# naver/deep-image-retrieval

Hardware: AMD Instinct MI355X
Metric: images/sec descriptor extraction (resnet101-GeM, 1024x1024) (higher is better)
Workload: dtype fp16p

## Files before the change

deep-image-retrieval_amd/csrc/conv_c3c1.hip:

```cpp
#include "dir_common.h"
#include "conv_device.h"
#include "conv_igemm.h"

namespace dir {

template <class DT, int P, bool DS, int P2, bool WP3 = false, bool WP1 = false>
__global__ void __launch_bounds__(512) conv_c3c1_kernel(const ConvArgs a) {
    static_assert(P == 64 || P == 128, "planes");
    static_assert(P2 == P || (P == 64 && P2 == 128), "conv1' width");
    static_assert(!DS || (P == 64 && P2 == 64), "the downsample form is layer1's: 64 + 64 input channels");
    static_assert((!WP3 && !WP1) || P == 64, "paired weights: layer1's seams");
    constexpr int KW = P + (DS ? 64 : 0);
    constexpr int KA = KW + (DS && WP3 ? 64 : 0);
    constexpr int C4 = 4 * P;
    constexpr int BM = 64, NT = 512;
    constexpr int CW = C4 / 8;
    constexpr int TA = CW / 32;
    constexpr int KSA = KA / 16;
    constexpr int KSW = KW / 16;
    constexpr int XBUF = BM * KA * 2;
    constexpr int NX = XBUF / 16 / NT;
    constexpr int EROW = 32 * 4 + 16;
    constexpr int EPI_OFF = 2 * XBUF;
    constexpr int OUT_OFF = EPI_OFF + 8 * 32 * EROW;
    constexpr int OUTB = BM * C4 * 2;
    constexpr int BIAS_OFF = OUT_OFF + OUTB;
    constexpr int KSB = (C4 / 2) / 16;
    typedef typename DT::frag_t frag_t;
    static_assert(NX >= 1 && XBUF % (16 * NT) == 0, "tile split");

    extern __shared__ __attribute__((aligned(16))) char smem[];

    const int tid = threadIdx.x;
    const int lane = tid & 63;
    const int wave = __builtin_amdgcn_readfirstlane(tid >> 6);
    const int lrow = lane & 31, lhi = lane >> 5;

    const __amdgpu_buffer_rsrc_t rsrc_x = buffer_rsrc(a.x, a.x_bytes);
    const __amdgpu_buffer_rsrc_t rsrc_x2 =
        buffer_rsrc(DS ? a.x2 : a.x, DS ? (uint32_t)((size_t)a.M * 128) : a.x_bytes);
    const __amdgpu_buffer_rsrc_t rsrc_x2l =
        buffer_rsrc(DS && WP3 ? a.x2_lo : a.x, DS && WP3 ? (uint32_t)((size_t)a.M * 128) : a.x_bytes);
    const uint32_t y_bytes = (uint32_t)((size_t)a.M * C4 * 2);
    const uint32_t y2_bytes = (uint32_t)((size_t)a.M * P2 * 2);
    const __amdgpu_buffer_rsrc_t rsrc_r = buffer_rsrc(a.res, y_bytes);
    const __amdgpu_buffer_rsrc_t rsrc_y = buffer_rsrc(a.y, y_bytes);
    const __amdgpu_buffer_rsrc_t rsrc_y2 = buffer_rsrc(a.y2, y2_bytes);

    const int mt = (a.M + BM - 1) / BM;
    const int per = gridDim.x;
    int tile = blockIdx.x;
    if (tile >= mt) return;
    Ovf<DT> ovf;
    const int n_wave = wave * CW;

    frag_t w3[TA][KSW], w3l[WP3 ? TA : 1][WP3 ? KSW : 1];
#pragma unroll
    for (int i = 0; i < TA; ++i)
#pragma unroll
        for (int ks = 0; ks < KSW; ++ks) {
            w3[i][ks] = *(const DIR_GLOBAL frag_t*)(a.w + (size_t)(n_wave + i * 32 + lrow) * KW + ks * 16 + 8 * lhi);
            if (WP3)
                w3l[i][ks] = *(const DIR_GLOBAL frag_t*)(a.w_lo + (size_t)(n_wave + i * 32 + lrow) * KW + ks * 16 + 8 * lhi);
        }
    constexpr bool WIDE = P2 == 128;
    const int nt = WIDE ? (wave & 3) : (wave & 1);
    const int kh = wave >> 2;
    const int jb = WIDE ? 0 : ((wave >> 1) & 1);
    frag_t w1[KSB], w1l[WP1 ? KSB : 1];
#pragma unroll
    for (int ks = 0; ks < KSB; ++ks) {
        w1[ks] = *(const DIR_GLOBAL frag_t*)(a.w2 + (size_t)(nt * 32 + lrow) * C4 + kh * (C4 / 2) + ks * 16 + 8 * lhi);
        if (WP1)
            w1l[ks] = *(const DIR_GLOBAL frag_t*)(a.w2_lo + (size_t)(nt * 32 + lrow) * C4 + kh * (C4 / 2) + ks * 16 + 8 * lhi);
    }
#pragma unroll
    for (int i = 0; i < TA; ++i)
#pragma unroll
        for (int ks = 0; ks < KSW; ++ks) {
// ... 7 lines not shown
    }

    const int spix = (tid >> 3) & 63, sslot = tid & 7;
    const int sdst = spix * 128 + ((sslot ^ ((spix >> 1) & 7)) << 4);
    const int lswz = (lane >> 1) & 7;
    const int lbase = lrow * 128;
    const int ecol = (lane & 3) * 8, erow = lane >> 2;
    float* const sbias3 = (float*)(smem + BIAS_OFF);
    float* const sbias1 = sbias3 + C4;
    for (int i = tid; i < C4; i += NT) sbias3[i] = a.bias[i];
    if (tid < P2) sbias1[tid] = a.bias2[tid];
    char* const ebase = smem + EPI_OFF + wave * (32 * EROW);
    char* const pbase = smem + EPI_OFF + (wave ^ 4) * (32 * EROW);
    char* const otile = smem + OUT_OFF;

    auto load_x = [&](int t, u32x4_t* xr) {
        const int m = t * BM + spix;
        const uint32_t base = m < a.M ? (uint32_t)((m * P + sslot * 8) * 2) : kOOB;
        if (DS) {
            xr[0] = __builtin_amdgcn_raw_buffer_load_b128(rsrc_x, base, 0, 0);
            xr[1] = __builtin_amdgcn_raw_buffer_load_b128(rsrc_x2, base, 0, 0);
            if (WP3) xr[NX - 1] = __builtin_amdgcn_raw_buffer_load_b128(rsrc_x2l, base, 0, 0);
        } else {
#pragma unroll
            for (int i = 0; i < NX; ++i) xr[i] = __builtin_amdgcn_raw_buffer_load_b128(rsrc_x, base, i * 128, 0);
        }
    };
    auto store_x = [&](const u32x4_t* xr, char* buf) {
#pragma unroll
        for (int i = 0; i < NX; ++i) *(u32x4_t*)(buf + i * (BM * 128) + sdst) = xr[i];
    };
    const uint32_t ncol2 = (uint32_t)((n_wave + ecol) * 2);
    auto row_off = [&](int m) { return m < a.M ? (uint32_t)m * (uint32_t)(C4 * 2) + ncol2 : kOOB; };
    auto load_res = [&](int t, int j, u32x4_t* r) {
#pragma unroll
        for (int i = 0; i < TA; ++i)
#pragma unroll
            for (int pass = 0; pass < 2; ++pass)
                r[i * 2 + pass] = __builtin_amdgcn_raw_buffer_load_b128(
                    rsrc_r, row_off(t * BM + j * 32 + pass * 16 + erow), i * 64, 0);
    };

    u32x4_t xr[NX];
    load_x(tile, xr);
    int cur = 0;
    u32x4_t rres0[TA * 2], rres1[TA * 2];
    if (!DS) load_res(tile, 0, rres0);
    store_x(xr, smem);
    __syncthreads();
    for (;;) {
        const bool more = tile + per < mt;
        const int next = more ? tile + per : tile;
        load_x(next, xr);
        const int m0 = tile * BM;
        if (!DS) load_res(tile, 1, rres1);
        const char* xb = smem + cur * XBUF;

#pragma unroll
        for (int j = 0; j < 2; ++j) {
            f32x16_t acc[TA];
#pragma unroll
            for (int i = 0; i < TA; ++i)
#pragma unroll
                for (int e = 0; e < 16; ++e) acc[i][e] = 0.f;
#pragma unroll
            for (int ks = 0; ks < KSA; ++ks) {
                const frag_t xf = *(const frag_t*)(xb + (ks >> 2) * (BM * 128) + j * (32 * 128) + lbase +
                                                   (((2 * (ks & 3) + lhi) ^ lswz) << 4));
                const int kw = ks < KSW ? ks : ks - 4;
#pragma unroll
                for (int i = 0; i < TA; ++i) {
                    acc[i] = DT::mfma32(w3[i][kw], xf, acc[i]);
                    if (WP3 && ks < KSW) acc[i] = DT::mfma32(w3l[i][ks], xf, acc[i]);
                }
                if ((ks & 3) == 3) __builtin_amdgcn_sched_barrier(0);
            }
            if (!DS) {
#pragma unroll
                for (int q = 0; q < TA * 2; ++q) {
                    if (j == 0) {
                        asm volatile("" : "+v"(rres0[q]));
                    } else {
                        asm volatile("" : "+v"(rres1[q]));
                    }
                }
            }
#pragma unroll
            for (int i = 0; i < TA; ++i) {
#pragma unroll
                for (int g = 0; g < 4; ++g) {
                    const f32x4_t v = {acc[i][4 * g + 0], acc[i][4 * g + 1], acc[i][4 * g + 2], acc[i][4 * g + 3]};
                    *(f32x4_t*)(ebase + lrow * EROW + (8 * g + 4 * lhi) * 4) = v;
                }
                wave_lds_sync();
                const float* const bz = sbias3 + n_wave + i * 32 + ecol;
                const f32x4_t b0 = *(const f32x4_t*)bz, b1 = *(const f32x4_t*)(bz + 4);
#pragma unroll
                for (int pass = 0; pass < 2; ++pass) {
                    const int mrow = pass * 16 + erow;
                    const f32x4_t f0 = *(const f32x4_t*)(ebase + mrow * EROW + ecol * 4);
                    const f32x4_t f1 = *(const f32x4_t*)(ebase + mrow * EROW + ecol * 4 + 16);
                    float v[8] = {f0[0] + b0[0], f0[1] + b0[1], f0[2] + b0[2], f0[3] + b0[3],
                                  f1[0] + b1[0], f1[1] + b1[1], f1[2] + b1[2], f1[3] + b1[3]};
                    if (!DS) {
                        const u32x4_t rv = j == 0 ? rres0[i * 2 + pass] : rres1[i * 2 + pass];
                        add_res8<DT>(v, rv);
                    }
                    if (a.relu) relu8(v);
                    u32x4_t ov;
#pragma unroll
                    for (int e = 0; e < 4; ++e) ov[e] = DT::pack(v[2 * e], v[2 * e + 1]);
                    __builtin_amdgcn_raw_buffer_store_b128(ov, rsrc_y, row_off(m0 + j * 32 + mrow), i * 64, 0);
                    ovf.see(ov);
                    const int n = n_wave + i * 32 + ecol, p = j * 32 + mrow;
                    *(u32x4_t*)(otile + (n >> 6) * (BM * 128) + p * 128 + ((((n & 63) >> 3) ^ ((p >> 1) & 7)) << 4)) = ov;
                }
                wave_lds_sync();
            }
            if (!DS && j == 0) load_res(next, 0, rres0);
        }
        __syncthreads();

        {
            constexpr int NJ = WIDE ? 2 : 1;
            f32x16_t acc1[NJ];
#pragma unroll
            for (int jj = 0; jj < NJ; ++jj)
#pragma unroll
                for (int e = 0; e < 16; ++e) acc1[jj][e] = 0.f;
#pragma unroll
            for (int ks = 0; ks < KSB; ++ks) {
                const int kb = kh * (C4 / 128) + (ks >> 2);
#pragma unroll
                for (int jj = 0; jj < NJ; ++jj) {
                    const int j = WIDE ? jj : jb;
                    const frag_t of = *(const frag_t*)(otile + kb * (BM * 128) + j * (32 * 128) + lbase +
                                                       (((2 * (ks & 3) + lhi) ^ lswz) << 4));
                    acc1[jj] = DT::mfma32(w1[ks], of, acc1[jj]);
                    if (WP1) acc1[jj] = DT::mfma32(w1l[ks], of, acc1[jj]);
                }
                if ((ks & 3) == 3) __builtin_amdgcn_sched_barrier(0);
            }
            const int give = WIDE ? (1 - kh) : 0;
            const bool gives = WIDE || kh == 1;
            const bool finishes = WIDE || kh == 0;
// ... 32 lines not shown
                    const int mrow = pass * 16 + erow;
                    const f32x4_t f0 = *(const f32x4_t*)(ebase + mrow * EROW + ecol * 4);
                    const f32x4_t f1 = *(const f32x4_t*)(ebase + mrow * EROW + ecol * 4 + 16);
                    float v[8] = {f0[0] + b0[0], f0[1] + b0[1], f0[2] + b0[2], f0[3] + b0[3],
                                  f1[0] + b1[0], f1[1] + b1[1], f1[2] + b1[2], f1[3] + b1[3]};
                    if (a.relu2) relu8(v);
                    const u32x4_t ov = pack8<DT>(v);
                    const int m = m0 + j * 32 + mrow;
                    const uint32_t off = m < a.M ? (uint32_t)m * (uint32_t)(P2 * 2) + (uint32_t)((nt * 32 + ecol) * 2) : kOOB;
                    __builtin_amdgcn_raw_buffer_store_b128(ov, rsrc_y2, off, 0, 0);
                    ovf.see(ov);
                }
            }
        }
        if (!more) break;
        store_x(xr, smem + (cur ^ 1) * XBUF);
        tile = next;
        cur ^= 1;
        __syncthreads();
    }
    ovf.flush(a.ovf);
}

bool conv_c3c1_admissible(const ConvArgs& a) {
    const bool ds = a.x2 != nullptr;
#ifdef DIR_EXPERIMENTS
    if (a.Cin == 256) return conv_seam3_admissible(a);
#endif
    return a.R == 1 && a.S == 1 && a.stride == 1 && a.pad == 0 && a.H == a.OH && a.W == a.OW &&
           (a.Cin == 64 || a.Cin == 128) && a.Cout == 4 * a.Cin && (ds ? (a.res == nullptr && a.Cin == 64 && a.Cin2 == 64)
                                                                       : a.res != nullptr) &&
           a.w2 != nullptr && a.bias2 != nullptr && a.y2 != nullptr &&
           (a.Cout2 == a.Cin || (!ds && a.Cin == 64 && a.Cout2 == 128)) && (long)a.M * a.Cout < (1L << 30) &&
           ((!a.w_lo && !a.w2_lo && !a.x2_lo) ||
            (a.Cin == 64 && a.w_lo && (a.w2_lo || a.Cout2 == 128) && (ds ? a.x2_lo != nullptr : a.x2_lo == nullptr)));
}

template <class DT, int P, bool DS, int P2 = P, bool WP3 = false, bool WP1 = false>
static hipError_t launch_c3c1(const ConvArgs& a, hipStream_t stream) {
    constexpr int XBUF = 64 * (P + (DS ? 64 : 0) + (DS && WP3 ? 64 : 0)) * 2;
    constexpr int LDS = 2 * XBUF + 8 * 32 * (32 * 4 + 16) + 64 * 4 * P * 2 + (4 * P + P2) * 4;
    static_assert(LDS <= 160 * 1024, "LDS budget");
    auto kern = conv_c3c1_kernel<DT, P, DS, P2, WP3, WP1>;
    static std::atomic<uint64_t> attr_done{0};
    if (hipError_t e = ensure_dynamic_lds((const void*)kern, LDS, attr_done); e != hipSuccess) return e;
    ConvArgs b = a;
    b.x_bytes = (uint32_t)((size_t)a.M * a.Cin * 2);
    const int mt = (a.M + 63) / 64;
    const int ncu = cu_count();
    hipLaunchKernelGGL(kern, dim3(mt < ncu ? mt : ncu), dim3(512), LDS, stream, b);
    return hipGetLastError();
}

hipError_t conv_c3c1_launch(const ConvArgs& a, int dtype, hipStream_t stream) {
#ifdef DIR_EXPERIMENTS
    if (a.Cin == 256) return conv_seam3_launch(a, dtype, stream);
#endif
    if (a.x2 && !env().no_c3c1lc && conv_c3c1ds_lc_admissible(a)) return conv_c3c1ds_lc_launch(a, dtype, stream);
    if (a.w_lo) {
        if (dtype != DIR_FP16) return hipErrorInvalidValue;
        if (a.x2) return a.w2_lo ? launch_c3c1<FP16, 64, true, 64, true, true>(a, stream) : hipErrorInvalidValue;
        if (a.Cout2 == 128)
            return a.w2_lo ? launch_c3c1<FP16, 64, false, 128, true, true>(a, stream)
                           : launch_c3c1<FP16, 64, false, 128, true, false>(a, stream);
        return a.w2_lo ? launch_c3c1<FP16, 64, false, 64, true, true>(a, stream) : hipErrorInvalidValue;
    }
    if (a.x2)
        return dtype == DIR_BF16 ? launch_c3c1<BF16, 64, true>(a, stream) : launch_c3c1<FP16, 64, true>(a, stream);
    if (a.Cin == 128)
        return dtype == DIR_BF16 ? launch_c3c1<BF16, 128, false>(a, stream) : launch_c3c1<FP16, 128, false>(a, stream);
    if (a.Cout2 == 128)
        return dtype == DIR_BF16 ? launch_c3c1<BF16, 64, false, 128>(a, stream) : launch_c3c1<FP16, 64, false, 128>(a, stream);
    return dtype == DIR_BF16 ? launch_c3c1<BF16, 64, false>(a, stream) : launch_c3c1<FP16, 64, false>(a, stream);
}

}
```

deep-image-retrieval_amd/csrc/conv_igemm.h:

```cpp
#pragma once
#include "dir_common.h"

namespace dir {

struct ConvArgs {
    const uint16_t* x;
    const uint16_t* w;
    const float* bias;
    const uint16_t* res;
    uint16_t* y;
    int B, H, W, Cin, OH, OW, Cout;
    int R, S, stride, pad, relu;
    int M;
    int Ktot;
    int T;
    int ksplit;
    float* partial;
    const uint16_t* w2;
    const float* bias2;
    uint16_t* y2;
    int Cout2, relu2;
    const uint16_t* x2;
    int Cin2;
    int H2, W2, stride2;
    uint32_t x2_bytes;
    int* ovf;
    const uint16_t* x_lo;
    const uint16_t* x2_lo;
    const uint16_t* w_lo;
    const uint16_t* w_pw;
    const uint16_t* w_s2;
    const uint16_t* w2_lo;
    const uint16_t* res_lo;
    uint16_t* y_lo;
    int tiles_m, tiles_n;
    uint32_t x_bytes, w_bytes;
    int rev_m;
    int no_xcd_map;
    int flat;
    uint32_t div_ohw_mul, div_ohw_shr;
    uint32_t div_ow_mul, div_ow_shr;
};

inline void fastdiv_init(uint32_t d, uint32_t& mul, uint32_t& shr) {
    if (d <= 1) {
        mul = 0;
        shr = 0;
        return;
    }
    uint32_t l = 0;
    while ((1ull << l) < d) ++l;
    mul = (uint32_t)(((1ull << (31 + l)) + d - 1) / d);
    shr = l - 1;
}
// ... 79 lines not shown
```

deep-image-retrieval_amd/csrc/dir_common.h:

```cpp
#pragma once
#include <hip/hip_runtime.h>
#include <stdint.h>
#include <string.h>
#include <atomic>
#include <string>

#include "../../include/dir_engine.h"

namespace dir {

typedef __attribute__((ext_vector_type(8))) __bf16 bf16x8_t;
typedef __attribute__((ext_vector_type(8))) _Float16 f16x8_t;
typedef __attribute__((ext_vector_type(16))) float f32x16_t;
typedef __attribute__((ext_vector_type(4))) float f32x4_t;
typedef __attribute__((ext_vector_type(4))) uint32_t u32x4_t;
typedef __attribute__((ext_vector_type(2))) uint32_t u32x2_t;
typedef __attribute__((ext_vector_type(2))) float f32x2_t;
typedef __attribute__((ext_vector_type(2))) __bf16 bf16x2_t;
typedef __attribute__((ext_vector_type(2))) _Float16 f16x2_t;

#define DIR_GLOBAL __attribute__((address_space(1)))
#define DIR_LDS __attribute__((address_space(3)))

void set_error(const std::string& msg);
int fail(int code, const std::string& msg);

#define DIR_HIP_CHECK(expr)                                                                \
    do {                                                                                   \
        hipError_t _e = (expr);                                                            \
        if (_e != hipSuccess)                                                              \
            return ::dir::fail(DIR_ERR_HIP, std::string(#expr) + ": " + hipGetErrorString(_e)); \
    } while (0)

struct Env {
    bool c3c1_off = false, c3c1_force = false;
    bool no_ds_seam = false, no_dual = false;
    bool rev_conv1 = false, rev_conv3 = false;
    bool unfused_stem = false, stem_v1 = false;
    bool no_patchlc = false, no_wreg = false, no_patchw = false, no_x3 = false, no_patchs = false;
    bool patchw_pack = false, no_patchw_pack = false;
    bool small_k2 = false;
    bool no_patchs2 = false;
    bool x3_k2048 = false;
    bool lc1x1 = false;
    bool no_c3c1lc = false;
    bool no_smallmap = false;
    bool no_wregd = false;
    bool no_patchw_lc = false;
    bool no_xcdmap = false;
    bool no_pair_patch = false, pair_acts = false;
    int pair_stages = 1;
    bool sim_v1 = false, sim_exact = false;
    bool experiments = false;
    bool no_inplace = false;
    bool no_stem_u8 = false;
    bool stem_pair_old = false;
    bool stem_u8_prep = false;
    bool stem_u8_wg8 = false;
    int stem_u8_seg = 0;
};
const Env& env();
void reload_env();

__host__ __device__ inline uint16_t f32_to_bf16_bits(float f) {
    uint32_t u;
    memcpy(&u, &f, 4);
    if ((u & 0x7fffffffu) > 0x7f800000u) return (uint16_t)((u >> 16) | 0x40);
    u += 0x7fffu + ((u >> 16) & 1u);
    return (uint16_t)(u >> 16);
}
__host__ __device__ inline float bf16_bits_to_f32(uint16_t h) {
    uint32_t u = ((uint32_t)h) << 16;
    float f;
    memcpy(&f, &u, 4);
    return f;
}
__host__ __device__ inline uint16_t f32_to_f16_bits(float f) {
    _Float16 h = (_Float16)f;
    uint16_t b;
    memcpy(&b, &h, 2);
    return b;
}
__host__ __device__ inline float f16_bits_to_f32(uint16_t b) {
    _Float16 h;
    memcpy(&h, &b, 2);
    return (float)h;
}
// ... 122 lines not shown
```

deep-image-retrieval_amd/csrc/engine.h:

```cpp
#pragma once
#include <map>
#include <string>
#include <vector>

#include "conv_f32.h"
#include "conv_igemm.h"
#include "pointwise.h"

namespace dir {

struct HostTensor {
    std::vector<int64_t> shape;
    std::vector<float> data;
};

struct ConvLayer {
    std::string name;
    std::string wkey;
    std::string bnprefix;
    int Cin = 0, Cout = 0, R = 1, S = 1, stride = 1, pad = 0;
    bool relu = false;
    bool stem = false;
    uint16_t* d_w = nullptr;
    float* d_wf = nullptr;
// ... 41 lines not shown
    std::vector<dir::ConvLayer> convs;
    std::vector<dir::BlockDef> blocks;
    int feat_dim = 0;
    int x4_dim = 0;
    int head_dim = 0;
    int x4_block = -1;
    int conv1x5 = -1, conv3c4 = -1;
    float gem_p = 3.f;
    float gem_p4 = 3.f;
    float* d_fc_w = nullptr;
    float* d_fc_b = nullptr;
    int* d_ovf = nullptr;
    uint16_t* d_stem_u8_w = nullptr;
    uint16_t* d_stem_u8_w_lo = nullptr;
    float* d_stem_u8_bias = nullptr;
    float* d_stem_u8_corr = nullptr;
    int fold_stem_u8(dir::ConvLayer& L, const float* w, const float* scale, const float* bias);
    bool profiling = false;
    bool prof_paused = false;
    std::vector<dir::ProfSlot> prof;
    size_t prof_used = 0;
    bool tuning = false;

    int build_graph();
    int finalize(int dtype);
    int plan(int B, int H, int W, dir::Plan* p) const;
    int forward(const void* img, int B, int H, int W, int fmt, float* desc_out, void* feat_out,
                int* fh, int* fw, int* fc, void* ws, size_t ws_bytes, hipStream_t stream);
    int forward_f32(const void* img, int B, int H, int W, int fmt, float* desc_out, void* feat_out, int* fh, int* fw,
                    int* fc, char* base, const dir::Plan& p, hipStream_t stream);
    int run_conv_f32(dir::ConvLayer& L, const float* x, const float* res, float* y, int B, int H, int W, int OH, int OW,
                     hipStream_t stream);
    int run_conv(dir::ConvLayer& L, const uint16_t* x, const uint16_t* res, uint16_t* y, int B,
                 int H, int W, int OH, int OW, hipStream_t stream, bool rev_m = false);
    int run_conv_pair(dir::ConvLayer& L, const uint16_t* x, const uint16_t* x_lo, const uint16_t* res,
                      const uint16_t* res_lo, uint16_t* y, uint16_t* y_lo, int B, int H, int W, int OH, int OW,
                      hipStream_t stream, const uint16_t* x2 = nullptr, const uint16_t* x2_lo = nullptr);
    int forward_pair_head(const void* img, int B, int H, int W, int fmt, char* base, const dir::Plan& p,
                          hipStream_t stream, uint16_t** cur, int* h, int* w, size_t* next_block);
    int forward_pair_stem(const void* img, int B, int H, int W, int fmt, char* base, const dir::Plan& p, hipStream_t stream);
    int run_seam(dir::ConvLayer& c3, dir::ConvLayer& c1, const uint16_t* t2, const uint16_t* res, uint16_t* y,
                 uint16_t* t1, int B, int H, int W, hipStream_t stream, int* used,
                 const uint16_t* block_in = nullptr, const uint16_t* block_in_lo = nullptr);
    int run_conv_dual(dir::ConvLayer& c3, const dir::ConvLayer& ds, const uint16_t* t2, const uint16_t* xin,
                      uint16_t* y, int B, int Hin, int Win, int OH, int OW, hipStream_t stream, int* used, bool dry);
    dir::Env sw;
    float* splitk_scratch = nullptr;
    int prof_begin(const std::string& name, const std::string& kernel, double flops, double bytes,
                   hipStream_t stream);
    int prof_end(hipStream_t stream);
    int overflow(hipStream_t stream, int* overflowed);
    void release();
};
```

deep-image-retrieval_amd/csrc/engine.hip:

```cpp
#include "engine.h"

#include <math.h>
#include <algorithm>

namespace dir {

static thread_local std::string g_err;
void set_error(const std::string& msg) { g_err = msg; }
int fail(int code, const std::string& msg) {
    g_err = msg;
    return code;
}
const char* last_error() { return g_err.c_str(); }


static Env read_env() {
    Env e;
    auto on = [](const char* k) { return getenv(k) != nullptr; };
    const char* mode = getenv("DIRTORCH_AMD_C3C1");
    e.c3c1_off = mode && mode[0] == '0';
    e.c3c1_force = mode && mode[0] == 'f';
    e.no_ds_seam = on("DIRTORCH_AMD_NO_DS_SEAM");
    e.no_dual = on("DIRTORCH_AMD_NO_DUAL");
    e.rev_conv1 = on("DIRTORCH_AMD_REV_CONV1");
    e.rev_conv3 = on("DIRTORCH_AMD_REV_CONV3");
    e.unfused_stem = on("DIRTORCH_AMD_UNFUSED_STEM");
    e.stem_v1 = on("DIRTORCH_AMD_STEM_V1");
    e.no_patchlc = on("DIRTORCH_AMD_NO_PATCHLC");
    e.no_wreg = on("DIRTORCH_AMD_NO_WREG");
    e.no_wregd = on("DIRTORCH_AMD_NO_WREGD");
    e.no_smallmap = on("DIRTORCH_AMD_NO_SMALLMAP");
    e.no_c3c1lc = on("DIRTORCH_AMD_NO_C3C1LC");
    e.lc1x1 = on("DIRTORCH_AMD_LC1X1");
    e.x3_k2048 = on("DIRTORCH_AMD_X3_K2048");
    e.no_patchs2 = on("DIRTORCH_AMD_NO_PATCHS2");
    e.small_k2 = on("DIRTORCH_AMD_SMALL_K2");
    e.patchw_pack = on("DIRTORCH_AMD_PATCHW_PACK");
    e.no_patchw_pack = on("DIRTORCH_AMD_NO_PATCHW_PACK");
    e.no_patchw = on("DIRTORCH_AMD_NO_PATCHW");
    e.no_x3 = on("DIRTORCH_AMD_NO_X3");
    e.no_patchs = on("DIRTORCH_AMD_NO_PATCHS");
    e.no_patchw_lc = on("DIRTORCH_AMD_NO_PATCHW_LC");
    e.no_xcdmap = on("DIRTORCH_AMD_NO_XCDMAP");
    e.no_pair_patch = on("DIRTORCH_AMD_NO_PAIR_PATCH");
    e.pair_acts = on("DIRTORCH_AMD_PAIR_ACTS");
    if (const char* s = getenv("DIRTORCH_AMD_PAIR_STAGES")) e.pair_stages = atoi(s);
    e.sim_v1 = on("DIRTORCH_AMD_SIM_V1");
    e.sim_exact = on("DIRTORCH_AMD_SIM_EXACT");
    e.experiments = on("DIRTORCH_AMD_EXPERIMENTS");
    e.no_inplace = on("DIRTORCH_AMD_NO_INPLACE");
    e.no_stem_u8 = on("DIRTORCH_AMD_NO_STEM_U8");
    e.stem_u8_wg8 = on("DIRTORCH_AMD_STEM_U8_WG8");
    e.stem_u8_prep = on("DIRTORCH_AMD_STEM_U8_PREP");
    e.stem_pair_old = on("DIRTORCH_AMD_STEM_PAIR_OLD");
    if (const char* s = getenv("DIRTORCH_AMD_STEM_U8_SEG")) e.stem_u8_seg = atoi(s);
    return e;
}
static Env g_env[2];
static std::atomic<int> g_env_cur{-1};
static std::atomic_flag g_env_lock = ATOMIC_FLAG_INIT;
static void publish_env() {
    while (g_env_lock.test_and_set(std::memory_order_acquire)) {
    }
    const int cur = g_env_cur.load(std::memory_order_relaxed);
    const int nxt = cur < 0 ? 0 : 1 - cur;
    g_env[nxt] = read_env();
    g_env_cur.store(nxt, std::memory_order_release);
    g_env_lock.clear(std::memory_order_release);
}
const Env& env() {
    int cur = g_env_cur.load(std::memory_order_acquire);
    if (cur < 0) {
        static const bool once = (publish_env(), true);
        (void)once;
        cur = g_env_cur.load(std::memory_order_acquire);
    }
    return g_env[cur];
}
void reload_env() { publish_env(); }

static inline size_t align_up(size_t v, size_t a = 256) { return (v + a - 1) / a * a; }

__global__ void fill_noise_kernel(uint16_t* p, long n, int dtype) {
// ... 404 lines not shown
    }
    p->splitk = take(kSplitKMaxBytes);
    p->pooled = take((size_t)B * head_dim * 4);
    p->fcout = take((size_t)B * std::max(desc.out_dim, head_dim) * 4);
    p->total = off;
    return DIR_OK;
}

int dir_engine::prof_begin(const std::string& name, const std::string& kernel, double flops,
                           double bytes, hipStream_t stream) {
    if (!profiling || prof_paused) return DIR_OK;
    if (prof_used == prof.size()) {
        ProfSlot s;
        DIR_HIP_CHECK(hipEventCreate(&s.start));
        DIR_HIP_CHECK(hipEventCreate(&s.stop));
        prof.push_back(s);
    }
    ProfSlot& s = prof[prof_used];
    s.name = name;
    s.kernel = kernel;
    s.flops = flops;
    s.bytes = bytes;
    DIR_HIP_CHECK(hipEventRecord(s.start, stream));
    return DIR_OK;
}
int dir_engine::prof_end(hipStream_t stream) {
    if (!profiling || prof_paused) return DIR_OK;
    DIR_HIP_CHECK(hipEventRecord(prof[prof_used].stop, stream));
    ++prof_used;
    return DIR_OK;
}

int dir_engine::run_conv(ConvLayer& L, const uint16_t* x, const uint16_t* res, uint16_t* y, int B,
                         int H, int W, int OH, int OW, hipStream_t stream, bool rev_m) {
    if (dtype == DIR_FP16P && L.d_w_lo && !L.stem)
        return run_conv_pair(L, x, nullptr, res, nullptr, y, nullptr, B, H, W, OH, OW, stream);
    ConvArgs a;
    memset(&a, 0, sizeof(a));
    a.rev_m = rev_m ? 1 : 0;
    a.x = x;
    a.w = L.d_w;
    a.w_s2 = L.d_w_s2;
    a.w_pw = env().no_patchw_pack ? nullptr : L.d_w_pw;
    a.bias = L.d_bias;
    a.res = res;
    a.y = y;
    a.B = B;
    a.H = H;
    a.W = W;
    a.OH = OH;
    a.OW = OW;
    a.Cout = L.Cout;
    if (L.stem) {
        a.Cin = 16;
        a.R = a.S = 4;
        a.stride = 1;
        a.pad = 2;
    } else {
        a.Cin = L.Cin;
        a.R = L.R;
        a.S = L.S;
        a.stride = L.stride;
        a.pad = L.pad;
    }
    a.relu = L.relu ? 1 : 0;
    a.ovf = d_ovf;
    a.partial = splitk_scratch;
    a.M = B * OH * OW;
    a.Ktot = a.R * a.S * a.Cin;
    a.T = a.Ktot / 64;
    const double macs = (double)a.M * L.Cout * (double)(L.R * L.S * L.Cin);
    const double bytes = 2.0 * ((double)B * H * W * a.Cin + (double)a.M * L.Cout * (res ? 2 : 1) +
                                (double)L.Cout * a.Ktot);

    int variant = -1;
    auto it = L.tuned.find(a.M);
    if (it != L.tuned.end()) variant = it->second;
    if (tuning && it == L.tuned.end()) {
        hipEvent_t e0, e1;
        DIR_HIP_CHECK(hipEventCreate(&e0));
        DIR_HIP_CHECK(hipEventCreate(&e1));
        float best = 1e30f;
        for (int v = 0; v < conv_variant_count(); ++v) {
            a.ksplit = 0;
            if (!conv_variant_admissible(v, a)) continue;
            a.ksplit = conv_splitk_factor(v, a);
            int rc = conv_launch(a, kdtype(), v, stream);
            if (rc != DIR_OK) return rc;
            float ms = 1e30f;
            for (int round = 0; round < 2; ++round) {
                DIR_HIP_CHECK(hipEventRecord(e0, stream));
                for (int rep = 0; rep < 3; ++rep) {
                    rc = conv_launch(a, kdtype(), v, stream);
                    if (rc != DIR_OK) return rc;
                }
                DIR_HIP_CHECK(hipEventRecord(e1, stream));
                DIR_HIP_CHECK(hipEventSynchronize(e1));
                float t = 0.f;
                DIR_HIP_CHECK(hipEventElapsedTime(&t, e0, e1));
                ms = t < ms ? t : ms;
            }
            if (ms < best) {
                best = ms;
                variant = v;
            }
        }
        (void)hipEventDestroy(e0);
        (void)hipEventDestroy(e1);
        L.tuned[a.M] = variant;
    }
    a.ksplit = 0;
    if (variant >= 0 && !conv_variant_admissible(variant, a)) {
        L.tuned.erase(a.M);
        variant = -1;
    }
    if (variant < 0) variant = conv_pick_variant(a);
    a.ksplit = conv_splitk_factor(variant, a);
    int rc = DIR_OK;
    if (profiling && !prof_paused)
        rc = prof_begin(L.name, std::string("conv_igemm<") + conv_variant(variant).name +
                                    (a.ksplit > 1 ? "/k" + std::to_string(a.ksplit) : "") + ">",
                        2.0 * macs, bytes, stream);
    if (rc != DIR_OK) return rc;
    rc = conv_launch(a, kdtype(), variant, stream);
    if (rc != DIR_OK) return rc;
    return prof_end(stream);
}

int dir_engine::run_conv_pair(ConvLayer& L, const uint16_t* x, const uint16_t* x_lo, const uint16_t* res,
                              const uint16_t* res_lo, uint16_t* y, uint16_t* y_lo, int B, int H, int W, int OH, int OW,
                              hipStream_t stream, const uint16_t* x2, const uint16_t* x2_lo) {
    if (!L.d_w_lo) return fail(DIR_ERR_STATE, "paired conv on a layer without a lo weight plane: " + L.name);
    if (x2 && !L.d_w_ds_lo) return fail(DIR_ERR_STATE, "two-source paired conv without concatenated weights: " + L.name);
    ConvArgs a;
    memset(&a, 0, sizeof(a));
    a.x = x;
    a.x_lo = x_lo;
    a.w = L.d_w;
    a.w_lo = L.d_w_lo;
    a.bias = L.d_bias;
    a.res = res;
    a.res_lo = res_lo;
    a.y = y;
    a.y_lo = y_lo;
    a.B = B;
    a.H = H;
    a.W = W;
// ... 114 lines not shown
        if (desc.bottleneck) {
            rc = run_conv_pair(convs[bd.conv1], x, x_lo, nullptr, nullptr, t1, t1_lo, B, h, w, h, w, stream);
            if (rc != DIR_OK) return rc;
            rc = run_conv_pair(convs[bd.conv2], t1, t1_lo, nullptr, nullptr, t2, t2_lo, B, h, w, oh, ow, stream);
            if (rc != DIR_OK) return rc;
            if (fuse_ds)
                rc = run_conv_pair(convs[bd.conv3], t2, t2_lo, nullptr, nullptr, pp[nxt], nullptr, B, oh, ow, oh, ow, stream,
                                   x, x_lo);
            else
                rc = run_conv_pair(convs[bd.conv3], t2, t2_lo, resid, resid_lo, pp[nxt], nullptr, B, oh, ow, oh, ow, stream);
            if (rc != DIR_OK) return rc;
        } else {
            rc = run_conv_pair(convs[bd.conv1], x, x_lo, nullptr, nullptr, t1, t1_lo, B, h, w, oh, ow, stream);
            if (rc != DIR_OK) return rc;
            rc = run_conv_pair(convs[bd.conv2], t1, t1_lo, resid, resid_lo, pp[nxt], nullptr, B, oh, ow, oh, ow, stream);
            if (rc != DIR_OK) return rc;
        }
        cur = nxt;
        h = oh;
        w = ow;
    }
    *cur_out = pp[cur];
    *h_out = h;
    *w_out = w;
    *next_block = nb;
    return DIR_OK;
}

static constexpr long kSeamMinTiles = 2048;
static constexpr long kSeam3MinTiles = 768;

int dir_engine::run_seam(ConvLayer& c3, ConvLayer& c1, const uint16_t* t2, const uint16_t* res, uint16_t* y,
                         uint16_t* t1, int B, int H, int W, hipStream_t stream, int* used,
                         const uint16_t* block_in, const uint16_t* block_in_lo) {
    *used = 0;
    if (sw.c3c1_off) return DIR_OK;
    ConvArgs a;
    memset(&a, 0, sizeof(a));
    a.x = t2;
    a.w = c3.d_w;
    a.w_lo = c3.d_w_lo;
    a.w2_lo = c1.d_w_lo;
    a.bias = c3.d_bias;
    a.res = res;
    if (block_in) {
        if (!c3.d_w_ds || c3.Cin != 64) return DIR_OK;
        a.w = c3.d_w_ds;
        a.w_lo = c3.d_w_ds_lo;
        a.bias = c3.d_bias_ds;
        a.res = nullptr;
        a.x2 = block_in;
        a.x2_lo = block_in_lo;
        a.Cin2 = 64;
        if ((c3.d_w_lo != nullptr) != (a.w_lo != nullptr)) return DIR_OK;
    }
    a.y = y;
    a.B = B;
    a.H = a.OH = H;
    a.W = a.OW = W;
    a.Cin = c3.Cin;
    a.Cout = c3.Cout;
    a.R = c3.R;
    a.S = c3.S;
    a.stride = c3.stride;
    a.pad = c3.pad;
    a.relu = c3.relu ? 1 : 0;
    a.M = B * H * W;
    a.Ktot = a.Cin;
    a.w2 = c1.d_w;
    a.bias2 = c1.d_bias;
    a.y2 = t1;
    a.Cout2 = c1.Cout;
    a.relu2 = c1.relu ? 1 : 0;
    a.ovf = d_ovf;
    if (c1.R != 1 || c1.S != 1 || c1.stride != 1 || c1.pad != 0 || c1.Cin != c3.Cout || !conv_c3c1_admissible(a))
        return DIR_OK;
    if (!sw.c3c1_force && (a.M + 63) / 64 < (a.Cin == 256 ? kSeam3MinTiles : kSeamMinTiles)) return DIR_OK;
    if (a.Cin == 256 && !sw.experiments) return DIR_OK;
    const double macs = (double)a.M * ((double)c3.Cout * (c3.Cin + a.Cin2) + (double)c1.Cout * c1.Cin);
    const double bytes = 2.0 * ((double)a.M * (c3.Cin + a.Cin2 * (block_in_lo ? 2 : 1) + (block_in ? 1.0 : 2.0) * c3.Cout + c1.Cout) +
                                (double)c3.Cout * (c3.Cin + a.Cin2) * (a.w_lo ? 2 : 1) + (double)c1.Cout * c1.Cin * (a.w2_lo ? 2 : 1));
    int rc = DIR_OK;
    if (profiling && !prof_paused)
        rc = prof_begin(c3.name.substr(0, c3.name.rfind('.')) + (block_in ? ".ds+c3c1" : ".c3c1"),
                        (c3.Cin == 256 ? "conv_seam3<" : "conv_c3c1<") + std::to_string(c3.Cin) + (block_in ? ",ds" : "") +
                            (a.w_lo ? ",wp>" : ">"),
                        2.0 * macs, bytes, stream);
    if (rc != DIR_OK) return rc;
    hipError_t e = conv_c3c1_launch(a, kdtype(), stream);
    if (e != hipSuccess) return fail(DIR_ERR_HIP, std::string("conv_c3c1 launch: ") + hipGetErrorString(e));
    *used = 1;
    return prof_end(stream);
}

int dir_engine::run_conv_dual(ConvLayer& c3, const ConvLayer& ds, const uint16_t* t2, const uint16_t* xin,
                              uint16_t* y, int B, int Hin, int Win, int OH, int OW, hipStream_t stream, int* used,
                              bool dry) {
    *used = 0;
    if (!c3.d_w_ds || sw.no_dual || c3.d_w_lo) return DIR_OK;
    ConvArgs a;
    memset(&a, 0, sizeof(a));
    a.x = t2;
    a.w = c3.d_w_ds;
    a.bias = c3.d_bias_ds;
    a.y = y;
    a.B = B;
    a.H = a.OH = OH;
    a.W = a.OW = OW;
    a.Cin = c3.Cin;
    a.Cout = c3.Cout;
    a.R = a.S = 1;
    a.stride = 1;
    a.relu = c3.relu ? 1 : 0;
    a.ovf = d_ovf;
    a.M = B * OH * OW;
    a.x2 = xin;
    a.Cin2 = ds.Cin;
    a.H2 = Hin;
    a.W2 = Win;
    a.stride2 = ds.stride;
    a.Ktot = a.Cin + a.Cin2;
    a.T = a.Ktot / 64;
    const int variant = conv_pick_dual_variant(a);
    if (variant < 0) return DIR_OK;
    *used = 1;
    if (dry) return DIR_OK;
    const double macs = (double)a.M * c3.Cout * (double)a.Ktot;
    const double bytes = 2.0 * ((double)a.M * (c3.Cin + ds.Cin + c3.Cout) + (double)c3.Cout * a.Ktot);
    int rc = DIR_OK;
    if (profiling && !prof_paused)
        rc = prof_begin(c3.name.substr(0, c3.name.rfind('.')) + ".ds+conv3",
                        std::string("conv_igemm<") + conv_variant(variant).name + "/dual>", 2.0 * macs, bytes, stream);
    if (rc != DIR_OK) return rc;
    rc = conv_launch(a, kdtype(), variant, stream);
    if (rc != DIR_OK) return rc;
    return prof_end(stream);
}

int dir_engine::forward(const void* img, int B, int H, int W, int fmt, float* desc_out,
                        void* feat_out, int* fh, int* fw, int* fc, void* ws, size_t ws_bytes,
                        hipStream_t stream) {
    if (!finalized) return fail(DIR_ERR_STATE, "forward before finalize");
    int cur_dev = -1;
    DIR_HIP_CHECK(hipGetDevice(&cur_dev));
    if (cur_dev != device)
        return fail(DIR_ERR_STATE, "forward: the current HIP device (" + std::to_string(cur_dev) +
                                       ") is not the engine's device (" + std::to_string(device) + ")");
    Plan p;
    int rc = plan(B, H, W, &p);
    if (rc != DIR_OK) return rc;
    if (!ws || ws_bytes < p.total)
        return fail(DIR_ERR_WORKSPACE, "workspace too small: need " + std::to_string(p.total) +
                                           " bytes, got " + std::to_string(ws_bytes));
// ... 35 lines not shown
        } else {
            const long n = (long)B * p.H2 * p.W2 * 16;
            hipLaunchKernelGGL(fill_noise_kernel, dim3((unsigned)((n + 255) / 256)), dim3(256), 0, stream,
                               s2d, n, kd);
            DIR_HIP_CHECK(hipGetLastError());
        }
        if (sw.unfused_stem) {
            rc = run_conv(convs[0], s2d, nullptr, stem, B, p.H2, p.W2, p.OH1, p.OW1, stream);
            if (rc != DIR_OK) return rc;
            rc = prof_begin("maxpool", "maxpool_3x3s2", 0,
                            2.0 * ((double)B * p.OH1 * p.OW1 * 64 + (double)B * p.PH * p.PW * 64), stream);
            if (rc != DIR_OK) return rc;
            rc = maxpool_3x3s2(stem, cur, B, p.OH1, p.OW1, 64, kd, stream);
            if (rc != DIR_OK) return rc;
            if ((rc = prof_end(stream)) != DIR_OK) return rc;
        } else {
            rc = prof_begin("conv1+maxpool", "stem_pool", 2.0 * B * p.OH1 * p.OW1 * 64.0 * 147.0,
                            2.0 * ((double)B * p.H2 * p.W2 * 16 + (double)B * p.PH * p.PW * 64 + 64 * 256),
                            stream);
            if (rc != DIR_OK) return rc;
            rc = stem_pool_launch(s2d, convs[0].d_w, convs[0].d_bias, cur, B, p.H2, p.W2, p.OH1, p.OW1,
                                  kd, stream, d_ovf);
            if (rc != DIR_OK) return rc;
            if ((rc = prof_end(stream)) != DIR_OK) return rc;
        }
        h = p.PH;
        w = p.PW;
    }

    uint16_t* const pp[2] = {(uint16_t*)(base + p.bufA), (uint16_t*)(base + p.bufB)};
    uint16_t* x4 = nullptr;
    int h4 = 0, w4 = 0;
    bool t1_ready = false;
    for (size_t bi = first_block; bi < blocks.size(); ++bi) {
        BlockDef& bd = blocks[bi];
        const int oh = conv_out(h, 3, bd.stride, 1), ow = conv_out(w, 3, bd.stride, 1);
        const bool keep = (int)bi == x4_block;
        nxt = keep ? (uint16_t*)(base + p.x4) : (cur == pp[0] ? pp[1] : pp[0]);
        if (!sw.no_inplace && desc.bottleneck && bd.down < 0 && !keep && !tuning && convs[bd.conv3].Cin >= 256) nxt = cur;
        const uint16_t* resid = cur;
        const bool seam_next = desc.bottleneck && bi + 1 < blocks.size() && !tuning;
        bool ds_in_seam = false;
        if (bd.down >= 0 && seam_next && convs[bd.conv3].d_w_ds && convs[bd.conv3].Cin == 64 &&
            convs[bd.down].Cin == 64 && convs[bd.down].stride == 1 && convs[blocks[bi + 1].conv1].Cout == 64 &&
            convs[blocks[bi + 1].conv1].Cin == convs[bd.conv3].Cout) {
            ds_in_seam = !sw.c3c1_off && !sw.no_ds_seam && (sw.c3c1_force || ((long)B * oh * ow + 63) / 64 >= kSeamMinTiles) &&
                         (long)B * oh * ow * convs[bd.conv3].Cout < (1L << 30);
        }
        int ds_dual = 0;
        if (bd.down >= 0 && !ds_in_seam && desc.bottleneck && !tuning && !cur_lo) {
            rc = run_conv_dual(convs[bd.conv3], convs[bd.down], t2, cur, nxt, B, h, w, oh, ow, stream, &ds_dual, true);
            if (rc != DIR_OK) return rc;
        }
        if (bd.down >= 0 && !ds_in_seam && !ds_dual) {
            rc = cur_lo ? run_conv_pair(convs[bd.down], cur, cur_lo, nullptr, nullptr, ds, nullptr, B, h, w, oh, ow, stream)
                        : run_conv(convs[bd.down], cur, nullptr, ds, B, h, w, oh, ow, stream);
            if (rc != DIR_OK) return rc;
            resid = ds;
        }
        if (desc.bottleneck) {
            if (!t1_ready) {
                rc = cur_lo ? run_conv_pair(convs[bd.conv1], cur, cur_lo, nullptr, nullptr, t1, nullptr, B, h, w, h, w, stream)
                            : run_conv(convs[bd.conv1], cur, nullptr, t1, B, h, w, h, w, stream, sw.rev_conv1);
                if (rc != DIR_OK) return rc;
            }
            t1_ready = false;
            rc = run_conv(convs[bd.conv2], t1, nullptr, t2, B, h, w, oh, ow, stream);
            if (rc != DIR_OK) return rc;
            int fused = 0;
            if (ds_dual) {
                rc = run_conv_dual(convs[bd.conv3], convs[bd.down], t2, cur, nxt, B, h, w, oh, ow, stream, &fused, false);
                if (rc != DIR_OK) return rc;
                if (!fused) return fail(DIR_ERR_STATE, "two-source conv declined a downsample it was promised");
                fused = 2;
            } else if (seam_next) {
                rc = run_seam(convs[bd.conv3], convs[blocks[bi + 1].conv1], t2, resid, nxt, t1, B, oh, ow, stream,
                              &fused, ds_in_seam ? cur : nullptr, ds_in_seam ? cur_lo : nullptr);
                if (rc != DIR_OK) return rc;
                if (ds_in_seam && !fused) return fail(DIR_ERR_STATE, "seam kernel declined a downsample it was promised");
            }
            if (fused == 1) {
                t1_ready = true;
            } else if (!fused) {
                rc = run_conv(convs[bd.conv3], t2, resid, nxt, B, oh, ow, oh, ow, stream, sw.rev_conv3);
                if (rc != DIR_OK) return rc;
            }
        } else {
            rc = run_conv(convs[bd.conv1], cur, nullptr, t1, B, h, w, oh, ow, stream);
            if (rc != DIR_OK) return rc;
            rc = run_conv(convs[bd.conv2], t1, resid, nxt, B, oh, ow, oh, ow, stream);
            if (rc != DIR_OK) return rc;
        }
        cur = nxt;
        cur_lo = nullptr;
        h = oh;
        w = ow;
        if (keep) {
            x4 = cur;
            h4 = h;
            w4 = w;
        }
    }
    if (feat_out) {
        DIR_HIP_CHECK(hipMemcpyAsync(feat_out, cur, (size_t)B * h * w * feat_dim * 2,
                                     hipMemcpyDeviceToDevice, stream));
        if (fh) *fh = h;
        if (fw) *fw = w;
        if (fc) *fc = feat_dim;
    }
    if (!desc_out) return DIR_OK;

    const bool fpn = x4 != nullptr;
// ... 217 lines not shown
```

Baseline: 2486.

## Write stage-closing seam output compactly at stride-2 positions for next downsample

When the last block of a stage feeds a stride-2 1x1 downsample, the fused conv3+conv1 seam kernel now stores only the even-row, even-column pixels of the block output into a compact buffer. The next block's downsample (plain or dual-source) then reads that buffer as a stride-1 input. This cuts global write traffic for the stage's final output by about 4x and shrinks the downsample's input reads. In exchange it adds per-row index division in the epilogue, a dry-run admissibility check, and extra state-consistency checks in the block loop.

Measured after the change: 2497 (median of 6 runs). About the same (+0.4%).

```diff
diff --git a/deep-image-retrieval_amd/csrc/conv_c3c1.hip b/deep-image-retrieval_amd/csrc/conv_c3c1.hip
--- a/deep-image-retrieval_amd/csrc/conv_c3c1.hip
+++ b/deep-image-retrieval_amd/csrc/conv_c3c1.hip
@@ -4,12 +4,13 @@
 
 namespace dir {
 
-template <class DT, int P, bool DS, int P2, bool WP3 = false, bool WP1 = false>
+template <class DT, int P, bool DS, int P2, bool WP3 = false, bool WP1 = false, bool SUB = false>
 __global__ void __launch_bounds__(512) conv_c3c1_kernel(const ConvArgs a) {
     static_assert(P == 64 || P == 128, "planes");
     static_assert(P2 == P || (P == 64 && P2 == 128), "conv1' width");
     static_assert(!DS || (P == 64 && P2 == 64), "the downsample form is layer1's: 64 + 64 input channels");
     static_assert((!WP3 && !WP1) || P == 64, "paired weights: layer1's seams");
+    static_assert(!SUB || (!DS && P2 == 2 * P), "compact block output: a stage-closing seam");
     constexpr int KW = P + (DS ? 64 : 0);
     constexpr int KA = KW + (DS && WP3 ? 64 : 0);
     constexpr int C4 = 4 * P;
@@ -44,7 +45,8 @@
     const uint32_t y_bytes = (uint32_t)((size_t)a.M * C4 * 2);
     const uint32_t y2_bytes = (uint32_t)((size_t)a.M * P2 * 2);
     const __amdgpu_buffer_rsrc_t rsrc_r = buffer_rsrc(a.res, y_bytes);
-    const __amdgpu_buffer_rsrc_t rsrc_y = buffer_rsrc(a.y, y_bytes);
+    const uint32_t sub_h = (uint32_t)(a.OH + 1) >> 1, sub_w = (uint32_t)(a.OW + 1) >> 1;
+    const __amdgpu_buffer_rsrc_t rsrc_y = buffer_rsrc(a.y, SUB ? (uint32_t)((size_t)a.B * sub_h * sub_w * C4 * 2) : y_bytes);
     const __amdgpu_buffer_rsrc_t rsrc_y2 = buffer_rsrc(a.y2, y2_bytes);
 
     const int mt = (a.M + BM - 1) / BM;
@@ -118,6 +120,16 @@
     };
     const uint32_t ncol2 = (uint32_t)((n_wave + ecol) * 2);
     auto row_off = [&](int m) { return m < a.M ? (uint32_t)m * (uint32_t)(C4 * 2) + ncol2 : kOOB; };
+    auto y_off = [&](int m) {
+        if (!SUB) return row_off(m);
+        const uint32_t mm = m < a.M ? (uint32_t)m : 0u;
+        const uint32_t b = fast_div(mm, a.div_ohw_mul, a.div_ohw_shr);
+        const uint32_t rem = mm - b * (uint32_t)(a.OH * a.OW);
+        const uint32_t oy = fast_div(rem, a.div_ow_mul, a.div_ow_shr);
+        const uint32_t ox = rem - oy * (uint32_t)a.OW;
+        const bool kept = m < a.M && ((oy | ox) & 1u) == 0;
+        return kept ? ((b * sub_h + (oy >> 1)) * sub_w + (ox >> 1)) * (uint32_t)(C4 * 2) + ncol2 : kOOB;
+    };
     auto load_res = [&](int t, int j, u32x4_t* r) {
 #pragma unroll
         for (int i = 0; i < TA; ++i)
@@ -161,6 +173,7 @@
                 }
                 if ((ks & 3) == 3) __builtin_amdgcn_sched_barrier(0);
             }
+            const uint32_t yo[2] = {y_off(m0 + j * 32 + erow), y_off(m0 + j * 32 + 16 + erow)};
             if (!DS) {
 #pragma unroll
                 for (int q = 0; q < TA * 2; ++q) {
@@ -196,7 +209,7 @@
                     u32x4_t ov;
 #pragma unroll
                     for (int e = 0; e < 4; ++e) ov[e] = DT::pack(v[2 * e], v[2 * e + 1]);
-                    __builtin_amdgcn_raw_buffer_store_b128(ov, rsrc_y, row_off(m0 + j * 32 + mrow), i * 64, 0);
+                    __builtin_amdgcn_raw_buffer_store_b128(ov, rsrc_y, yo[pass], i * 64, 0);
                     ovf.see(ov);
                     const int n = n_wave + i * 32 + ecol, p = j * 32 + mrow;
                     *(u32x4_t*)(otile + (n >> 6) * (BM * 128) + p * 128 + ((((n & 63) >> 3) ^ ((p >> 1) & 7)) << 4)) = ov;
@@ -295,27 +308,38 @@
                                                                        : a.res != nullptr) &&
            a.w2 != nullptr && a.bias2 != nullptr && a.y2 != nullptr &&
            (a.Cout2 == a.Cin || (!ds && a.Cin == 64 && a.Cout2 == 128)) && (long)a.M * a.Cout < (1L << 30) &&
+           (a.y_sub == 0 || (a.y_sub == 2 && !ds && a.Cout2 == 2 * a.Cin && a.B > 0 && a.M == a.B * a.OH * a.OW)) &&
            ((!a.w_lo && !a.w2_lo && !a.x2_lo) ||
             (a.Cin == 64 && a.w_lo && (a.w2_lo || a.Cout2 == 128) && (ds ? a.x2_lo != nullptr : a.x2_lo == nullptr)));
 }
 
-template <class DT, int P, bool DS, int P2 = P, bool WP3 = false, bool WP1 = false>
+template <class DT, int P, bool DS, int P2 = P, bool WP3 = false, bool WP1 = false, bool SUB = false>
 static hipError_t launch_c3c1(const ConvArgs& a, hipStream_t stream) {
     constexpr int XBUF = 64 * (P + (DS ? 64 : 0) + (DS && WP3 ? 64 : 0)) * 2;
     constexpr int LDS = 2 * XBUF + 8 * 32 * (32 * 4 + 16) + 64 * 4 * P * 2 + (4 * P + P2) * 4;
     static_assert(LDS <= 160 * 1024, "LDS budget");
-    auto kern = conv_c3c1_kernel<DT, P, DS, P2, WP3, WP1>;
+    auto kern = conv_c3c1_kernel<DT, P, DS, P2, WP3, WP1, SUB>;
     static std::atomic<uint64_t> attr_done{0};
     if (hipError_t e = ensure_dynamic_lds((const void*)kern, LDS, attr_done); e != hipSuccess) return e;
     ConvArgs b = a;
     b.x_bytes = (uint32_t)((size_t)a.M * a.Cin * 2);
+    if (SUB) {
+        fastdiv_init((uint32_t)(a.OH * a.OW), b.div_ohw_mul, b.div_ohw_shr);
+        fastdiv_init((uint32_t)a.OW, b.div_ow_mul, b.div_ow_shr);
+    }
     const int mt = (a.M + 63) / 64;
     const int ncu = cu_count();
     hipLaunchKernelGGL(kern, dim3(mt < ncu ? mt : ncu), dim3(512), LDS, stream, b);
     return hipGetLastError();
 }
 
+template <class DT, bool WP3 = false, bool WP1 = false>
+static hipError_t launch_c3c1_wide(const ConvArgs& a, hipStream_t stream) {
+    return a.y_sub ? launch_c3c1<DT, 64, false, 128, WP3, WP1, true>(a, stream) : launch_c3c1<DT, 64, false, 128, WP3, WP1>(a, stream);
+}
+
 hipError_t conv_c3c1_launch(const ConvArgs& a, int dtype, hipStream_t stream) {
+    if (a.y_sub && !conv_c3c1_admissible(a)) return hipErrorInvalidValue;
 #ifdef DIR_EXPERIMENTS
     if (a.Cin == 256) return conv_seam3_launch(a, dtype, stream);
 #endif
@@ -324,8 +348,7 @@
         if (dtype != DIR_FP16) return hipErrorInvalidValue;
         if (a.x2) return a.w2_lo ? launch_c3c1<FP16, 64, true, 64, true, true>(a, stream) : hipErrorInvalidValue;
         if (a.Cout2 == 128)
-            return a.w2_lo ? launch_c3c1<FP16, 64, false, 128, true, true>(a, stream)
-                           : launch_c3c1<FP16, 64, false, 128, true, false>(a, stream);
+            return a.w2_lo ? launch_c3c1_wide<FP16, true, true>(a, stream) : launch_c3c1_wide<FP16, true, false>(a, stream);
         return a.w2_lo ? launch_c3c1<FP16, 64, false, 64, true, true>(a, stream) : hipErrorInvalidValue;
     }
     if (a.x2)
@@ -333,7 +356,7 @@
     if (a.Cin == 128)
         return dtype == DIR_BF16 ? launch_c3c1<BF16, 128, false>(a, stream) : launch_c3c1<FP16, 128, false>(a, stream);
     if (a.Cout2 == 128)
-        return dtype == DIR_BF16 ? launch_c3c1<BF16, 64, false, 128>(a, stream) : launch_c3c1<FP16, 64, false, 128>(a, stream);
+        return dtype == DIR_BF16 ? launch_c3c1_wide<BF16>(a, stream) : launch_c3c1_wide<FP16>(a, stream);
     return dtype == DIR_BF16 ? launch_c3c1<BF16, 64, false>(a, stream) : launch_c3c1<FP16, 64, false>(a, stream);
 }
 
diff --git a/deep-image-retrieval_amd/csrc/conv_igemm.h b/deep-image-retrieval_amd/csrc/conv_igemm.h
--- a/deep-image-retrieval_amd/csrc/conv_igemm.h
+++ b/deep-image-retrieval_amd/csrc/conv_igemm.h
@@ -20,6 +20,7 @@
     const float* bias2;
     uint16_t* y2;
     int Cout2, relu2;
+    int y_sub;
     const uint16_t* x2;
     int Cin2;
     int H2, W2, stride2;
diff --git a/deep-image-retrieval_amd/csrc/dir_common.h b/deep-image-retrieval_amd/csrc/dir_common.h
--- a/deep-image-retrieval_amd/csrc/dir_common.h
+++ b/deep-image-retrieval_amd/csrc/dir_common.h
@@ -53,6 +53,7 @@
     bool sim_v1 = false, sim_exact = false;
     bool experiments = false;
     bool no_inplace = false;
+    bool no_compact_out = false;
     bool no_stem_u8 = false;
     bool stem_pair_old = false;
     bool stem_u8_prep = false;
diff --git a/deep-image-retrieval_amd/csrc/engine.h b/deep-image-retrieval_amd/csrc/engine.h
--- a/deep-image-retrieval_amd/csrc/engine.h
+++ b/deep-image-retrieval_amd/csrc/engine.h
@@ -97,7 +97,7 @@
     int run_conv_f32(dir::ConvLayer& L, const float* x, const float* res, float* y, int B, int H, int W, int OH, int OW,
                      hipStream_t stream);
     int run_conv(dir::ConvLayer& L, const uint16_t* x, const uint16_t* res, uint16_t* y, int B,
-                 int H, int W, int OH, int OW, hipStream_t stream, bool rev_m = false);
+                 int H, int W, int OH, int OW, hipStream_t stream, bool rev_m = false, bool x_compact = false);
     int run_conv_pair(dir::ConvLayer& L, const uint16_t* x, const uint16_t* x_lo, const uint16_t* res,
                       const uint16_t* res_lo, uint16_t* y, uint16_t* y_lo, int B, int H, int W, int OH, int OW,
                       hipStream_t stream, const uint16_t* x2 = nullptr, const uint16_t* x2_lo = nullptr);
@@ -106,9 +106,10 @@
     int forward_pair_stem(const void* img, int B, int H, int W, int fmt, char* base, const dir::Plan& p, hipStream_t stream);
     int run_seam(dir::ConvLayer& c3, dir::ConvLayer& c1, const uint16_t* t2, const uint16_t* res, uint16_t* y,
                  uint16_t* t1, int B, int H, int W, hipStream_t stream, int* used,
-                 const uint16_t* block_in = nullptr, const uint16_t* block_in_lo = nullptr);
+                 const uint16_t* block_in = nullptr, const uint16_t* block_in_lo = nullptr, int y_sub = 0, bool dry = false);
     int run_conv_dual(dir::ConvLayer& c3, const dir::ConvLayer& ds, const uint16_t* t2, const uint16_t* xin,
-                      uint16_t* y, int B, int Hin, int Win, int OH, int OW, hipStream_t stream, int* used, bool dry);
+                      uint16_t* y, int B, int Hin, int Win, int OH, int OW, hipStream_t stream, int* used, bool dry,
+                      bool x_compact = false);
     dir::Env sw;
     float* splitk_scratch = nullptr;
     int prof_begin(const std::string& name, const std::string& kernel, double flops, double bytes,
diff --git a/deep-image-retrieval_amd/csrc/engine.hip b/deep-image-retrieval_amd/csrc/engine.hip
--- a/deep-image-retrieval_amd/csrc/engine.hip
+++ b/deep-image-retrieval_amd/csrc/engine.hip
@@ -49,6 +49,7 @@
     e.sim_exact = on("DIRTORCH_AMD_SIM_EXACT");
     e.experiments = on("DIRTORCH_AMD_EXPERIMENTS");
     e.no_inplace = on("DIRTORCH_AMD_NO_INPLACE");
+    e.no_compact_out = on("DIRTORCH_AMD_NO_COMPACT_OUT");
     e.no_stem_u8 = on("DIRTORCH_AMD_NO_STEM_U8");
     e.stem_u8_wg8 = on("DIRTORCH_AMD_STEM_U8_WG8");
     e.stem_u8_prep = on("DIRTORCH_AMD_STEM_U8_PREP");
@@ -519,7 +520,9 @@
 }
 
 int dir_engine::run_conv(ConvLayer& L, const uint16_t* x, const uint16_t* res, uint16_t* y, int B,
-                         int H, int W, int OH, int OW, hipStream_t stream, bool rev_m) {
+                         int H, int W, int OH, int OW, hipStream_t stream, bool rev_m, bool x_compact) {
+    if (x_compact && (L.R != 1 || L.S != 1 || L.pad != 0 || L.stem || (dtype == DIR_FP16P && L.d_w_lo)))
+        return fail(DIR_ERR_STATE, "compact input: " + L.name + " is not a plain 1x1 convolution");
     if (dtype == DIR_FP16P && L.d_w_lo && !L.stem)
         return run_conv_pair(L, x, nullptr, res, nullptr, y, nullptr, B, H, W, OH, OW, stream);
     ConvArgs a;
@@ -557,7 +560,7 @@
     a.Ktot = a.R * a.S * a.Cin;
     a.T = a.Ktot / 64;
     const double macs = (double)a.M * L.Cout * (double)(L.R * L.S * L.Cin);
-    const double bytes = 2.0 * ((double)B * H * W * a.Cin + (double)a.M * L.Cout * (res ? 2 : 1) +
+    const double bytes = 2.0 * ((double)B * (x_compact ? OH * OW : H * W) * a.Cin + (double)a.M * L.Cout * (res ? 2 : 1) +
                                 (double)L.Cout * a.Ktot);
 
     int variant = -1;
@@ -600,6 +603,13 @@
     if (variant >= 0 && !conv_variant_admissible(variant, a)) {
         L.tuned.erase(a.M);
         variant = -1;
+    }
+    if (x_compact) {
+        if (variant < 0) variant = conv_pick_variant(a);
+        a.H = OH;
+        a.W = OW;
+        a.stride = 1;
+        if (!conv_variant_admissible(variant, a)) variant = -1;
     }
     if (variant < 0) variant = conv_pick_variant(a);
     a.ksplit = conv_splitk_factor(variant, a);
@@ -780,7 +790,7 @@
 
 int dir_engine::run_seam(ConvLayer& c3, ConvLayer& c1, const uint16_t* t2, const uint16_t* res, uint16_t* y,
                          uint16_t* t1, int B, int H, int W, hipStream_t stream, int* used,
-                         const uint16_t* block_in, const uint16_t* block_in_lo) {
+                         const uint16_t* block_in, const uint16_t* block_in_lo, int y_sub, bool dry) {
     *used = 0;
     if (sw.c3c1_off) return DIR_OK;
     ConvArgs a;
@@ -803,6 +813,7 @@
         if ((c3.d_w_lo != nullptr) != (a.w_lo != nullptr)) return DIR_OK;
     }
     a.y = y;
+    a.y_sub = y_sub;
     a.B = B;
     a.H = a.OH = H;
     a.W = a.OW = W;
@@ -825,8 +836,14 @@
         return DIR_OK;
     if (!sw.c3c1_force && (a.M + 63) / 64 < (a.Cin == 256 ? kSeam3MinTiles : kSeamMinTiles)) return DIR_OK;
     if (a.Cin == 256 && !sw.experiments) return DIR_OK;
+    if (dry) {
+        *used = 1;
+        return DIR_OK;
+    }
     const double macs = (double)a.M * ((double)c3.Cout * (c3.Cin + a.Cin2) + (double)c1.Cout * c1.Cin);
-    const double bytes = 2.0 * ((double)a.M * (c3.Cin + a.Cin2 * (block_in_lo ? 2 : 1) + (block_in ? 1.0 : 2.0) * c3.Cout + c1.Cout) +
+    const double y_pix = y_sub == 2 ? (double)B * ((H + 1) / 2) * ((W + 1) / 2) : (double)a.M;
+    const double bytes = 2.0 * ((double)a.M * (c3.Cin + a.Cin2 * (block_in_lo ? 2 : 1) + (block_in ? 0.0 : 1.0) * c3.Cout + c1.Cout) +
+                                y_pix * c3.Cout +
                                 (double)c3.Cout * (c3.Cin + a.Cin2) * (a.w_lo ? 2 : 1) + (double)c1.Cout * c1.Cin * (a.w2_lo ? 2 : 1));
     int rc = DIR_OK;
     if (profiling && !prof_paused)
@@ -843,7 +860,7 @@
 
 int dir_engine::run_conv_dual(ConvLayer& c3, const ConvLayer& ds, const uint16_t* t2, const uint16_t* xin,
                               uint16_t* y, int B, int Hin, int Win, int OH, int OW, hipStream_t stream, int* used,
-                              bool dry) {
+                              bool dry, bool x_compact) {
     *used = 0;
     if (!c3.d_w_ds || sw.no_dual || c3.d_w_lo) return DIR_OK;
     ConvArgs a;
@@ -864,9 +881,9 @@
     a.M = B * OH * OW;
     a.x2 = xin;
     a.Cin2 = ds.Cin;
-    a.H2 = Hin;
-    a.W2 = Win;
-    a.stride2 = ds.stride;
+    a.H2 = x_compact ? OH : Hin;
+    a.W2 = x_compact ? OW : Win;
+    a.stride2 = x_compact ? 1 : ds.stride;
     a.Ktot = a.Cin + a.Cin2;
     a.T = a.Ktot / 64;
     const int variant = conv_pick_dual_variant(a);
@@ -968,6 +985,7 @@
     uint16_t* x4 = nullptr;
     int h4 = 0, w4 = 0;
     bool t1_ready = false;
+    bool cur_compact = false;
     for (size_t bi = first_block; bi < blocks.size(); ++bi) {
         BlockDef& bd = blocks[bi];
         const int oh = conv_out(h, 3, bd.stride, 1), ow = conv_out(w, 3, bd.stride, 1);
@@ -984,13 +1002,17 @@
                          (long)B * oh * ow * convs[bd.conv3].Cout < (1L << 30);
         }
         int ds_dual = 0;
+        const bool in_compact = cur_compact;
+        cur_compact = false;
+        if (in_compact && (bd.down < 0 || ds_in_seam || cur_lo || !t1_ready || !desc.bottleneck))
+            return fail(DIR_ERR_STATE, "a block other than a stage's first was handed a compact input");
         if (bd.down >= 0 && !ds_in_seam && desc.bottleneck && !tuning && !cur_lo) {
-            rc = run_conv_dual(convs[bd.conv3], convs[bd.down], t2, cur, nxt, B, h, w, oh, ow, stream, &ds_dual, true);
+            rc = run_conv_dual(convs[bd.conv3], convs[bd.down], t2, cur, nxt, B, h, w, oh, ow, stream, &ds_dual, true, in_compact);
             if (rc != DIR_OK) return rc;
         }
         if (bd.down >= 0 && !ds_in_seam && !ds_dual) {
             rc = cur_lo ? run_conv_pair(convs[bd.down], cur, cur_lo, nullptr, nullptr, ds, nullptr, B, h, w, oh, ow, stream)
-                        : run_conv(convs[bd.down], cur, nullptr, ds, B, h, w, oh, ow, stream);
+                        : run_conv(convs[bd.down], cur, nullptr, ds, B, h, w, oh, ow, stream, false, in_compact);
             if (rc != DIR_OK) return rc;
             resid = ds;
         }
@@ -1004,16 +1026,31 @@
             rc = run_conv(convs[bd.conv2], t1, nullptr, t2, B, h, w, oh, ow, stream);
             if (rc != DIR_OK) return rc;
             int fused = 0;
+            int y_sub = 0;
+            if (seam_next && !ds_dual && !ds_in_seam && !sw.no_compact_out && !keep && nxt != cur && blocks[bi + 1].down >= 0 &&
+                blocks[bi + 1].stride == 2) {
+                const ConvLayer& nd = convs[blocks[bi + 1].down];
+                if (nd.R == 1 && nd.S == 1 && nd.stride == 2 && nd.pad == 0 && nd.Cin == convs[bd.conv3].Cout &&
+                    !(dtype == DIR_FP16P && nd.d_w_lo)) {
+                    int would = 0;
+                    rc = run_seam(convs[bd.conv3], convs[blocks[bi + 1].conv1], t2, resid, nxt, t1, B, oh, ow, stream, &would,
+                                  nullptr, nullptr, 2, true);
+                    if (rc != DIR_OK) return rc;
+                    if (would) y_sub = 2;
+                }
+            }
             if (ds_dual) {
-                rc = run_conv_dual(convs[bd.conv3], convs[bd.down], t2, cur, nxt, B, h, w, oh, ow, stream, &fused, false);
+                rc = run_conv_dual(convs[bd.conv3], convs[bd.down], t2, cur, nxt, B, h, w, oh, ow, stream, &fused, false, in_compact);
                 if (rc != DIR_OK) return rc;
                 if (!fused) return fail(DIR_ERR_STATE, "two-source conv declined a downsample it was promised");
                 fused = 2;
             } else if (seam_next) {
                 rc = run_seam(convs[bd.conv3], convs[blocks[bi + 1].conv1], t2, resid, nxt, t1, B, oh, ow, stream,
-                              &fused, ds_in_seam ? cur : nullptr, ds_in_seam ? cur_lo : nullptr);
+                              &fused, ds_in_seam ? cur : nullptr, ds_in_seam ? cur_lo : nullptr, y_sub);
                 if (rc != DIR_OK) return rc;
                 if (ds_in_seam && !fused) return fail(DIR_ERR_STATE, "seam kernel declined a downsample it was promised");
+                if (y_sub && !fused) return fail(DIR_ERR_STATE, "seam kernel declined a compact block output it was promised");
+                cur_compact = y_sub != 0;
             }
             if (fused == 1) {
                 t1_ready = true;
```
